# VisionDepth/VisionDepth3D

Hardware: AMD Instinct MI355X
Metric: stereo-pairs/sec end-to-end (depth+warp+fill+mux) (higher is better)
Workload: dtype f32

## Files before the change

### include/vd3d.h

```cpp
#ifndef VD3D_H
#define VD3D_H

#include <stddef.h>
#include <stdint.h>

#ifdef __cplusplus
extern "C" {
#endif

#define VD3D_ABI_VERSION 6

typedef enum vd3d_status {
  VD3D_OK = 0,
  VD3D_E_INVALID = -1,
  VD3D_E_HIP = -2,
  VD3D_E_NOMEM = -3,
  VD3D_E_UNSUPPORTED = -4
} vd3d_status;

typedef enum vd3d_format {
  VD3D_FMT_HALF_SBS = 0,
  VD3D_FMT_FULL_SBS = 1,
  VD3D_FMT_VR = 2,
  VD3D_FMT_ANAGLYPH = 3,
// ... 165 lines not shown
int vd3d_conv3x3_c64_f16(vd3d_ctx* ctx, const void* x_nhwc, int H, int W, const void* w_frag, const float* bias, const float* slope_or_null,
                         void* y_nhwc);
int vd3d_conv3x3_head_f16(vd3d_ctx* ctx, const void* x_nhwc3, int H, int W, const float* w27x64, const float* bias, const float* slope_or_null,
                          void* y_nhwc64);
int vd3d_esr_tail_f32(vd3d_ctx* ctx, const void* t_nhwc64, const void* x_nhwc3, int H, int W, int r, float* out_planar);

int vd3d_depth_handoff(vd3d_ctx* ctx, const float* pred, int B, int ph, int pw, int H, int W, int invert, uint8_t* out_gray);

typedef enum vd3d_dtype { VD3D_DT_BF16 = 0, VD3D_DT_F32 = 1, VD3D_DT_F16 = 2  } vd3d_dtype;

int vd3d_depth_preprocess(vd3d_ctx* ctx, const uint8_t* frames_bgr, int B, int H, int W, int th, int tw,
                          const float* mean3_host, const float* std3_host, int dtype, void* out_nhwc);

int vd3d_add_layernorm(vd3d_ctx* ctx, int dtype, const void* x, const void* y_or_null, const void* gamma, const void* beta,
                       float eps, int64_t rows, int cols, void* out_sum, void* out_norm);

enum { VD3D_GEMM_EPI_NONE = 0, VD3D_GEMM_EPI_GELU = 1 };
enum { VD3D_X3_BF16X3 = 0, VD3D_X3_FP16X2 = 1 };
int64_t vd3d_gemm_x3_weight_bytes(int N, int K, int mode);
int vd3d_gemm_x3_pack_weights(vd3d_ctx* ctx, const float* W, int N, int K, int mode, void* image);
int vd3d_gemm_x3(vd3d_ctx* ctx, const float* X, int64_t M, int K, const void* w_image, int N, int mode, const float* bias_or_null, int epilogue, float* Y);
int64_t vd3d_attention_x3_workspace_bytes(int B, int T, int H, int D, int mode);
int vd3d_attention_x3(vd3d_ctx* ctx, const float* qkv, int B, int T, int H, int D, float scale, int mode, void* workspace, int64_t workspace_bytes, float* out);

int64_t vd3d_conv3x3_x2_weight_bytes(int Cin, int Cout);
int vd3d_conv3x3_x2_pack_weights(vd3d_ctx* ctx, const float* W, int Cin, int Cout, void* image);
int vd3d_conv3x3_x2(vd3d_ctx* ctx, const float* X, int B, int H, int W, int Cin, const void* w_image, int Cout, float* Y);

int vd3d_upsample_bilinear_nhwc(vd3d_ctx* ctx, int dtype, const void* in, void* out, int B, int ih, int iw, int oh, int ow, int C);

int vd3d_nhwc_bias_act_f32(vd3d_ctx* ctx, const float* y, const float* bias_or_null, const float* r1_or_null, const float* r2_or_null, int relu,
                           int64_t n_pix, int C, float* out, float* relu_out_or_null);
int vd3d_upsample_bilinear_bias_nhwc_f32(vd3d_ctx* ctx, const float* in, const float* bias, float* out, int B, int ih, int iw, int oh, int ow, int C);
int vd3d_dpt_head_tail_f32(vd3d_ctx* ctx, const float* y, const float* b2, const float* w3, float b3, float scale, int64_t n_pix, int C, float* out);

int vd3d_depth_to_space_bias_nhwc_f32(vd3d_ctx* ctx, const float* y, const float* bias_or_null, int B, int H, int W, int s, int C, float* out);

typedef enum vd3d_preview {
  VD3D_PREVIEW_INTERLACED = 0,
  VD3D_PREVIEW_HSBS = 1,
  VD3D_PREVIEW_LR_DIFF = 2,
  VD3D_PREVIEW_FEATHER_BLEND = 3,
  VD3D_PREVIEW_RED_BLUE = 4
} vd3d_preview;
int vd3d_preview_image(vd3d_ctx* ctx, int type, const uint8_t* left_bgr, const uint8_t* right_bgr, int h, int w, uint8_t* out_bgr);
int vd3d_preview_heatmap(vd3d_ctx* ctx, int type, const float* shift_map, int h, int w, const uint8_t* lut_bgr_dev, uint8_t* out_bgr);
// ... 25 lines not shown
```

### visiondepth3d_amd/_lib.py

```python
from __future__ import annotations

import ctypes as C
import os

from . import _abi
from ._abi import FrameScalars, RenderParams, ShiftParams, State

_HERE = os.path.dirname(os.path.abspath(__file__))
LIB_PATH = os.environ.get("VD3D_LIB_PATH") or os.path.join(_HERE, "libvd3d_hip.so")

EXPORTS = (
    "vd3d_abi_version", "vd3d_last_error", "vd3d_shift_params_default", "vd3d_render_params_default",
    "vd3d_ctx_create", "vd3d_ctx_destroy", "vd3d_sync", "vd3d_ctx_stream", "vd3d_ctx_set_stream", "vd3d_ctx_pixel_stream", "vd3d_ctx_pixel_stream_k",
    "vd3d_state_reset", "vd3d_state_new_clip", "vd3d_state_export", "vd3d_state_import", "vd3d_state_planes",
    "vd3d_last_scalars", "vd3d_pixel_shift", "vd3d_render_frame", "vd3d_render_frame_blank", "vd3d_depth_handoff", "vd3d_heal_missing_pixels", "vd3d_preview_heatmap", "vd3d_preview_arrows", "vd3d_conv3x3_c64_f16", "vd3d_conv3x3_head_f16", "vd3d_esr_tail_f32", "vd3d_nv12_to_bgr", "vd3d_bgr_to_nv12", "vd3d_resize_cubic_u8", "vd3d_resize_area_u8", "vd3d_resize_linear_u8", "vd3d_format_3d_output", "vd3d_esr_preprocess", "vd3d_esr_postprocess", "vd3d_add_weighted_u8", "vd3d_rife_preprocess", "vd3d_rife_postprocess",
    "vd3d_shard_begin", "vd3d_shard_pixels", "vd3d_shard_pixels_blank", "vd3d_tdf_plane_export", "vd3d_tdf_plane_import", "vd3d_set_pixel_overlap", "vd3d_join_pixels", "vd3d_wait_pixels", "vd3d_finish_frame", "vd3d_quantiles",
    "vd3d_subject_depth", "vd3d_shard2_p0", "vd3d_shard2_set_crops", "vd3d_shard2_p1", "vd3d_shard2_p1_batch", "vd3d_shard2_r1", "vd3d_shard2_p3", "vd3d_shard2_p3_batch", "vd3d_shard2_r2", "vd3d_depth_preprocess", "vd3d_add_layernorm", "vd3d_gemm_x3_weight_bytes", "vd3d_gemm_x3_pack_weights", "vd3d_gemm_x3", "vd3d_attention_x3_workspace_bytes", "vd3d_attention_x3", "vd3d_conv3x3_x2_weight_bytes", "vd3d_conv3x3_x2_pack_weights", "vd3d_conv3x3_x2", "vd3d_upsample_bilinear_nhwc", "vd3d_nhwc_bias_act_f32", "vd3d_upsample_bilinear_bias_nhwc_f32", "vd3d_dpt_head_tail_f32", "vd3d_depth_to_space_bias_nhwc_f32", "vd3d_preview_image", "vd3d_detect_black_bars", "vd3d_stream_copy", "vd3d_torch_math", "vd3d_torch_math_aten", "vd3d_debug_gaussian_kernel1d", "vd3d_debug_exp_torch", "vd3d_set_profiling", "vd3d_last_stage_ms", "vd3d_stage_calls",
    "vd3d_debug_planes", "vd3d_debug_tune",
)

_lib = None


class Vd3dError(RuntimeError):
    def __init__(self, code, msg):
        super().__init__(f"libvd3d_hip error {code}: {msg}")
        self.code = code


def lib():
    global _lib
    if _lib is not None:
        return _lib
    if not os.path.exists(LIB_PATH):
        raise ImportError(f"{LIB_PATH} not built: run `python -c 'import __graft_entry__ as g; g.build()'` "
                          "(hipcc --offload-arch=gfx950). There is no CPU fallback.")
    L = C.CDLL(LIB_PATH)
    vp, i32, f32p, u8p = C.c_void_p, C.c_int, C.c_void_p, C.c_void_p
    L.vd3d_abi_version.restype = i32
    L.vd3d_last_error.restype = C.c_char_p
# ... 41 lines not shown
    L.vd3d_esr_postprocess.argtypes = [vp, f32p, i32, i32, i32, i32, i32, i32, i32, u8p, C.c_longlong]
    L.vd3d_rife_preprocess.argtypes = [vp, i32, u8p, u8p, i32, i32, i32, vp]
    L.vd3d_rife_postprocess.argtypes = [vp, f32p, i32, i32, i32, u8p]
    L.vd3d_add_weighted_u8.argtypes = [vp, u8p, C.c_double, u8p, C.c_double, C.c_double, C.c_longlong, u8p]
    L.vd3d_finish_frame.argtypes = [vp, u8p, u8p, f32p, i32, i32, C.POINTER(RenderParams), C.c_double, i32, i32, u8p]
    L.vd3d_quantiles.argtypes = [vp, f32p, C.c_int64, C.POINTER(C.c_float), i32, C.POINTER(C.c_float)]
    L.vd3d_subject_depth.argtypes = [vp, f32p, i32, i32, C.POINTER(C.c_float)]
    L.vd3d_shard2_p0.argtypes = [vp, vp, vp, vp]
    L.vd3d_shard2_set_crops.argtypes = [vp, vp, i32]
    L.vd3d_shard2_p1.argtypes = [vp, vp, vp, i32, vp, i32, i32, vp]
    L.vd3d_shard2_p1_batch.argtypes = [vp, vp, vp, i32, vp, i32, i32, i32, vp]
    L.vd3d_shard2_p3_batch.argtypes = [vp, i32, i32, i32, vp, vp]
    L.vd3d_shard2_r1.argtypes = [vp, vp, i32]
    L.vd3d_shard2_p3.argtypes = [vp, i32, i32, vp, vp]
    L.vd3d_shard2_r2.argtypes = [vp, vp, C.POINTER(C.c_int), C.POINTER(C.c_uint8), i32, vp]
    L.vd3d_depth_preprocess.argtypes = [vp, vp, i32, i32, i32, i32, i32, C.POINTER(C.c_float), C.POINTER(C.c_float), i32, vp]
    L.vd3d_gemm_x3_weight_bytes.argtypes = [i32, i32, i32]
    L.vd3d_gemm_x3_weight_bytes.restype = C.c_int64
    L.vd3d_gemm_x3_pack_weights.argtypes = [vp, vp, i32, i32, i32, vp]
    L.vd3d_gemm_x3.argtypes = [vp, vp, C.c_int64, i32, vp, i32, i32, vp, i32, vp]
    L.vd3d_attention_x3_workspace_bytes.argtypes = [i32, i32, i32, i32, i32]
    L.vd3d_attention_x3_workspace_bytes.restype = C.c_int64
    L.vd3d_attention_x3.argtypes = [vp, vp, i32, i32, i32, i32, C.c_float, i32, vp, C.c_int64, vp]
    L.vd3d_conv3x3_x2_weight_bytes.argtypes = [i32, i32]
    L.vd3d_conv3x3_x2_weight_bytes.restype = C.c_int64
    L.vd3d_conv3x3_x2_pack_weights.argtypes = [vp, vp, i32, i32, vp]
    L.vd3d_conv3x3_x2.argtypes = [vp, vp, i32, i32, i32, i32, vp, i32, vp]
    L.vd3d_add_layernorm.argtypes = [vp, i32, vp, vp, vp, vp, C.c_float, C.c_int64, i32, vp, vp]
    L.vd3d_upsample_bilinear_nhwc.argtypes = [vp, i32, vp, vp, i32, i32, i32, i32, i32, i32]
    L.vd3d_nhwc_bias_act_f32.argtypes = [vp, vp, vp, vp, vp, i32, C.c_int64, i32, vp, vp]
    L.vd3d_upsample_bilinear_bias_nhwc_f32.argtypes = [vp, vp, vp, vp, i32, i32, i32, i32, i32, i32]
    L.vd3d_dpt_head_tail_f32.argtypes = [vp, vp, vp, vp, C.c_float, C.c_float, C.c_int64, i32, vp]
    L.vd3d_depth_to_space_bias_nhwc_f32.argtypes = [vp, vp, vp, i32, i32, i32, i32, i32, vp]
    L.vd3d_preview_image.argtypes = [vp, i32, vp, vp, i32, i32, vp]
    L.vd3d_detect_black_bars.argtypes = [vp, vp, i32, i32, C.POINTER(C.c_int), C.POINTER(C.c_int)]
    L.vd3d_stream_copy.argtypes = [vp, vp, vp, C.c_size_t]
    L.vd3d_torch_math.argtypes = [vp, i32, vp, C.c_float, vp, C.c_longlong]
    L.vd3d_torch_math_aten.argtypes = [vp, i32, vp, C.c_double, vp, C.c_longlong, i32]
    L.vd3d_debug_gaussian_kernel1d.argtypes = [i32, C.c_float, vp]
    L.vd3d_debug_exp_torch.argtypes = [vp, vp, C.c_longlong]
    L.vd3d_debug_tune.argtypes = [i32, i32]
    L.vd3d_set_profiling.argtypes = [vp, i32]
    L.vd3d_last_stage_ms.argtypes = [vp, C.c_char_p]
    L.vd3d_last_stage_ms.restype = C.c_float
    L.vd3d_stage_calls.argtypes = [vp, C.c_char_p]
    L.vd3d_stage_calls.restype = C.c_long
# ... 20 lines not shown
```

### visiondepth3d_amd/csrc/vd3d_api.hip

```cpp
#include <hip/hip_runtime.h>

#include <cmath>
#include <cstdarg>
#include <cstddef>
#include <cstdio>
#include <cstring>
#include <cstdlib>
#include <map>
#include <string>
#include <vector>

#include "vd3d_kernels.h"

#define VD3D_EXPORT extern "C" __attribute__((visibility("default")))

static thread_local char g_err[512] = "";
static int set_err(int code, const char* fmt, ...) {
  va_list ap;
  va_start(ap, fmt);
  vsnprintf(g_err, sizeof g_err, fmt, ap);
  va_end(ap);
  return code;
}
#define HIPCHK(x)                                                                                     \
// ... 1303 lines not shown
VD3D_EXPORT int vd3d_conv3x3_x2_pack_weights(vd3d_ctx* c, const float* W, int Cin, int Cout, void* image) {
  if (!c || !W || !image) return set_err(VD3D_E_INVALID, "bad argument");
  if (!vd_launch_conv3x3_x2_pack(c->stream, W, Cin, Cout, image))
    return set_err(VD3D_E_UNSUPPORTED, "conv3x3_x2: C_in %d must be a positive multiple of 16 and C_out %d one of 64, 128", Cin, Cout);
  HIPCHK(hipGetLastError());
  return 0;
}

VD3D_EXPORT int vd3d_conv3x3_x2(vd3d_ctx* c, const float* X, int B, int H, int W, int Cin, const void* w_image, int Cout, float* Y) {
  if (!c || !X || !w_image || !Y) return set_err(VD3D_E_INVALID, "bad argument");
  if (!vd_launch_conv3x3_x2(c->stream, X, B, H, W, Cin, w_image, Cout, Y))
    return set_err(VD3D_E_UNSUPPORTED, "conv3x3_x2: C_in %d (multiple of 16), C_out %d (64 | 128), B %d <= 65535, 16-byte aligned input and image", Cin, Cout, B);
  HIPCHK(hipGetLastError());
  return 0;
}

VD3D_EXPORT int64_t vd3d_attention_x3_workspace_bytes(int B, int T, int H, int D, int mode) { return (int64_t)vd_attn_x3_workspace_bytes(B, T, H, D, mode); }

VD3D_EXPORT int vd3d_attention_x3(vd3d_ctx* c, const float* qkv, int B, int T, int H, int D, float scale, int mode, void* workspace, int64_t workspace_bytes, float* out) {
  if (!c || !qkv || !workspace || !out) return set_err(VD3D_E_INVALID, "bad argument");
  const long long need = vd_attn_x3_workspace_bytes(B, T, H, D, mode);
  if (need < 0) return set_err(VD3D_E_UNSUPPORTED, "attention_x3: head size %d not built (64), an unknown mode %d or an empty shape (B %d T %d H %d)", D, mode, B, T, H);
  if (workspace_bytes < need) return set_err(VD3D_E_INVALID, "attention_x3: workspace of %lld bytes, %lld needed", (long long)workspace_bytes, need);
  if (!vd_launch_attn_x3(c->stream, qkv, B, T, H, D, scale, workspace, out, mode))
    return set_err(VD3D_E_UNSUPPORTED, "attention_x3: qkv / workspace / out must be 16-byte aligned, B * H <= 65535");
  HIPCHK(hipGetLastError());
  return 0;
}

VD3D_EXPORT int64_t vd3d_gemm_x3_weight_bytes(int N, int K, int mode) { return (int64_t)vd_gemm_x3_weight_bytes(N, K, mode); }

VD3D_EXPORT int vd3d_gemm_x3_pack_weights(vd3d_ctx* c, const float* W, int N, int K, int mode, void* image) {
  if (!c || !W || !image) return set_err(VD3D_E_INVALID, "bad argument");
  if (!vd_launch_gemm_x3_pack_w(c->stream, W, N, K, image, mode)) return set_err(VD3D_E_UNSUPPORTED, "gemm_x3: K %d must be a positive multiple of 16 (N %d), mode %d in {0, 1}", K, N, mode);
  HIPCHK(hipGetLastError());
  return 0;
}

VD3D_EXPORT int vd3d_gemm_x3(vd3d_ctx* c, const float* X, int64_t M, int K, const void* w_image, int N, int mode, const float* bias_or_null, int epilogue, float* Y) {
  if (!c || !X || !w_image || !Y || M < 1) return set_err(VD3D_E_INVALID, "bad argument");
  if (epilogue != VD3D_GEMM_EPI_NONE && epilogue != VD3D_GEMM_EPI_GELU) return set_err(VD3D_E_INVALID, "gemm_x3: unknown epilogue %d", epilogue);
  if (!vd_launch_gemm_x3(c->stream, X, (long long)M, K, w_image, N, bias_or_null, epilogue, Y, mode))
    return set_err(VD3D_E_UNSUPPORTED, "gemm_x3: K %d must be a positive multiple of 16, mode %d in {0, 1}, X and the weight image 16-byte aligned", K, mode);
  HIPCHK(hipGetLastError());
  return 0;
}

VD3D_EXPORT int vd3d_upsample_bilinear_nhwc(vd3d_ctx* c, int dtype, const void* in, void* out, int B, int ih, int iw, int oh, int ow, int C) {
// ... 205 lines not shown
```

### visiondepth3d_amd/csrc/vd3d_attn.hip

```cpp
#include "vd3d_dev.h"
#include "vd3d_kernels.h"

typedef short at_bf8 __attribute__((ext_vector_type(8)));
typedef float at_f16 __attribute__((ext_vector_type(16)));
typedef uint32_t at_u4 __attribute__((ext_vector_type(4)));

#define AT_D 64
#define AT_BQ 256
#define AT_BK 64
#define AT_NT 512
#define AT_NTERM(MODE) ((MODE) == 0 ? 3 : 2)
#define AT_TILE(MODE) (4 * AT_NTERM(MODE) * 2 * 64 * 16)
#define AT_STAGE(MODE) (2 * AT_TILE(MODE))
#define AT_NSTAGE 3
#define AT_LDS(MODE) (AT_NSTAGE * AT_STAGE(MODE))
#define AT_QBLK(MODE) (4 * AT_NTERM(MODE) * 2 * 32)
#define AT_QKV_SCALE 16.0f
#define AT_P_SCALE 1024.0f
#define AT_OP 272

struct vd_at_args {
  int B, H, T;
  int nq32, nkv, nqb;
  float c;
// ... 255 lines not shown
  __builtin_amdgcn_s_barrier();

  const float l_tot = l_half + __shfl_xor(l_half, 32, 64);
  const float inv = MODE == 1 ? 1.0f / (l_tot * (AT_P_SCALE * AT_QKV_SCALE)) : 1.0f / l_tot;
  uint8_t* ow = at_lds + wave * (32 * AT_OP);
#pragma unroll
  for (int dm = 0; dm < 2; ++dm)
#pragma unroll
    for (int g = 0; g < 4; ++g) {
      const float4 v4 = {oacc[dm][4 * g] * inv, oacc[dm][4 * g + 1] * inv, oacc[dm][4 * g + 2] * inv, oacc[dm][4 * g + 3] * inv};
      *reinterpret_cast<float4*>(ow + li * AT_OP + (32 * dm + 8 * g + 4 * kh) * 4) = v4;
    }
  asm volatile("s_waitcnt lgkmcnt(0)" ::: "memory");
  const int b = bh / a.H, h = bh - b * a.H;
#pragma unroll
  for (int i = 0; i < 8; ++i) {
    const int row = i * 4 + (lane >> 4), c4 = lane & 15;
    const int q = q0 + row;
    const float4 v4 = *reinterpret_cast<const float4*>(ow + row * AT_OP + c4 * 16);
    if (q < a.T) *reinterpret_cast<float4*>(out + (((size_t)b * a.T + q) * a.H + h) * AT_D + c4 * 4) = v4;
  }
}

static bool at_mode_ok(int mode) { return mode == 0 || mode == 1; }
long long vd_attn_x3_workspace_bytes(int B, int T, int H, int D, int mode) {
  if (B < 1 || T < 1 || H < 1 || D != AT_D || !at_mode_ok(mode)) return -1;
  const long long nq32 = (T + 31) / 32, nkv = (T + AT_BK - 1) / AT_BK;
  const long long qblk = mode == 0 ? AT_QBLK(0) : AT_QBLK(1), tile = mode == 0 ? AT_TILE(0) : AT_TILE(1);
  return (long long)B * H * (nq32 * qblk * 16 + 2 * nkv * tile);
}

template <int MODE>
static bool at_launch(hipStream_t s, const float* qkv, int B, int T, int H, float scale, void* ws, float* out) {
  static bool attr_set = false;
  if (!attr_set) {
    if (hipFuncSetAttribute(reinterpret_cast<const void*>(k_attn_bf16x3<MODE>), hipFuncAttributeMaxDynamicSharedMemorySize, AT_LDS(MODE)) != hipSuccess) return false;
    attr_set = true;
  }
  vd_at_args a;
  a.B = B; a.H = H; a.T = T;
  a.nq32 = (T + 31) / 32; a.nkv = (T + AT_BK - 1) / AT_BK; a.nqb = (T + AT_BQ - 1) / AT_BQ;
  a.c = scale * 1.44269504088896340736f;
  if (MODE == 1) a.c *= 1.0f / (AT_QKV_SCALE * AT_QKV_SCALE);
  uint4* Qimg = reinterpret_cast<uint4*>(ws);
  uint4* Kimg = Qimg + (size_t)B * H * a.nq32 * AT_QBLK(MODE);
  uint4* Vimg = Kimg + (size_t)B * H * a.nkv * (AT_TILE(MODE) / 16);
  const int rows_max = a.nkv * 64 > a.nq32 * 32 ? a.nkv * 64 : a.nq32 * 32;
  hipLaunchKernelGGL(k_attn_x3_prep<MODE>, dim3((unsigned)((rows_max * 8 + 255) / 256), (unsigned)(B * H), 3), dim3(256), 0, s, qkv, a, Qimg, Kimg, Vimg);
  const int groups = (B * H + 7) / 8;
  hipLaunchKernelGGL(k_attn_bf16x3<MODE>, dim3((unsigned)(8 * groups * a.nqb)), dim3(AT_NT), AT_LDS(MODE), s, Qimg, Kimg, Vimg, out, a);
  return true;
}

bool vd_launch_attn_x3(hipStream_t s, const float* qkv, int B, int T, int H, int D, float scale, void* ws, float* out, int mode) {
  if (vd_attn_x3_workspace_bytes(B, T, H, D, mode) < 0) return false;
  if ((reinterpret_cast<uintptr_t>(qkv) & 15) || (reinterpret_cast<uintptr_t>(ws) & 15) || (reinterpret_cast<uintptr_t>(out) & 15)) return false;
  if ((long long)B * H > 65535) return false;
  return mode == 0 ? at_launch<0>(s, qkv, B, T, H, scale, ws, out) : at_launch<1>(s, qkv, B, T, H, scale, ws, out);
}
```

### visiondepth3d_amd/csrc/vd3d_kernels.h

```cpp
#pragma once
#include <hip/hip_runtime.h>

#include "vd3d_work.h"

enum { VD_ST_A0 = 0, VD_ST_B0, VD_ST_A1, VD_ST_B1, VD_ST_A2, VD_ST_B2,
       VD_ST_AQ, VD_ST_BQ, VD_ST_BS };
#define PL_KMAX_HOST 129
#define DF_RMAX_HOST 15

#define VD_ETAB 8
struct vd_stage_args {
  int stage;
  int have_eye;
  int W, H;
  long long n_eye;
  long long n_crop;
  double ipd_factor;
  int shard;
  int shard_idx;
  float* q_out;
  long long* m_out;
  const int* crop_tab;
  const float* etab;
  int dbg;
// ... 136 lines not shown
                               const vd_finish_consts& fc, const vd_dev_work* w, float focal_override, int use_override,
                               int bar_width, int bar_side, uint8_t* L_out, uint8_t* R_out, const float* wtab);
#define VD_D4_WTAB_FLOATS (4 * 31 * 32)
bool vd_launch_sharp_fit(hipStream_t s, const uint8_t* gL, const uint8_t* gR, const vd3d_render_params& p, const vd_finish_consts& fc, uint8_t* out);
void vd_launch_sharp_mux(hipStream_t s, const uint8_t* gL, const uint8_t* gR, const vd3d_render_params& p,
                         const vd_finish_consts& fc, uint8_t* out, int presharp_pitch = 0, bool identity_fit = false);
void vd_launch_stream_copy(hipStream_t s, const void* src, void* dst, size_t bytes);
void vd_launch_interp_planes(hipStream_t s, const float* src, int C, int ih, int iw, float* dst, int oh, int ow, int premult);
void vd_launch_torch_math_aten(hipStream_t s, int op, const float* x, double p, float* out, long long n, int threads);
void vd_launch_torch_math(hipStream_t s, int op, const float* x, float p, float* out, long long n);
void vd_launch_blank_eye(hipStream_t s, const uint8_t* src, int h, int w, const vd_dev_work* wk, uint8_t* dst);

bool vd_launch_preview(hipStream_t s, int type, const uint8_t* L, const uint8_t* R, int h, int w, uint8_t* out);
bool vd_launch_depth_prep(hipStream_t s, const uint8_t* frames, int B, int H, int W, int th, int tw, const float mean[3],
                          const float stdv[3], int dtype, void* out_nhwc);
long long vd_gemm_x3_weight_bytes(int N, int K, int mode);
bool vd_launch_gemm_x3_pack_w(hipStream_t s, const float* W, int N, int K, void* img, int mode);
bool vd_launch_gemm_x3(hipStream_t s, const float* X, long long M, int K, const void* wimg, int N, const float* bias, int epilogue, float* Y, int mode);
long long vd_conv3x3_x2_weight_bytes(int Cin, int Cout);
bool vd_launch_conv3x3_x2_pack(hipStream_t s, const float* W, int Cin, int Cout, void* img);
bool vd_launch_conv3x3_x2(hipStream_t s, const float* X, int B, int H, int W, int Cin, const void* wimg, int Cout, float* Y);
long long vd_attn_x3_workspace_bytes(int B, int T, int H, int D, int mode);
bool vd_launch_attn_x3(hipStream_t s, const float* qkv, int B, int T, int H, int D, float scale, void* ws, float* out, int mode);
bool vd_launch_add_layernorm(hipStream_t s, int dtype, const void* x, const void* y, const void* gamma, const void* beta, float eps,
                             long long rows, int cols, void* out_sum, void* out_norm);
bool vd_launch_upsample_bilinear_nhwc(hipStream_t s, int dtype, const void* in, void* out, int B, int ih, int iw, int oh, int ow, int C);
bool vd_launch_bias_act_f32(hipStream_t s, const float* y, const float* bias, const float* r1, const float* r2, int relu, long long n_pix, int C,
                            float* out, float* relu_out);
bool vd_launch_upsample_bilinear_bias_nhwc_f32(hipStream_t s, const float* in, const float* bias, float* out, int B, int ih, int iw, int oh, int ow, int C);
bool vd_launch_head_tail_f32(hipStream_t s, const float* y, const float* b2, const float* w3, float b3, float scale, long long n_pix, int C, float* out);
bool vd_launch_depth_to_space_bias_f32(hipStream_t s, const float* y, const float* bias, int B, int H, int W, int f, int C, float* out);
void vd_launch_depth_handoff(hipStream_t s, const float* pred, int B, int ph, int pw, int H, int W, int invert, uint32_t* mm,
                             uint8_t* out);

bool vd_launch_finish_fused(hipStream_t s, const uint8_t* L, const uint8_t* R, const float* dn, int eh, int ew,
                            const vd3d_render_params& p, const vd_finish_consts& fc, const vd_dev_work* w, float focal,
                            int use_override, int bar_w, int bar_s, uint8_t* out, int dense, const float* w2_dev);

bool vd_launch_conv3x3_c64_f16(hipStream_t s, const void* x, int H, int W, const void* wfrag, const float* bias, const float* slope_or_null, void* y);
void vd_launch_conv3x3_head_f16(hipStream_t s, const void* x, int H, int W, const float* w27, const float* bias, const float* slope_or_null, void* y);
void vd_launch_esr_tail_f32(hipStream_t s, const void* t, const void* x, int H, int W, int r, float* out);
void vd_launch_nv12_to_bgr(hipStream_t s, const uint8_t* y, const uint8_t* uv, int h, int w, long long y_pitch, long long uv_pitch, uint8_t* out);
void vd_launch_bgr_to_nv12(hipStream_t s, const uint8_t* bgr, int h, int w, uint8_t* y, uint8_t* uv, long long y_pitch, long long uv_pitch);
bool vd_launch_preview_heatmap(hipStream_t s, int type, const float* shift, int h, int w, const uint8_t* lut_dev, uint32_t* mm, uint8_t* out);
void vd_launch_preview_arrows(hipStream_t s, const uint8_t* left, const float* shift, int h, int w, uint8_t* out);
bool vd_launch_resize_cubic_u8(hipStream_t s, const uint8_t* src, int sh, int sw, int cn, uint8_t* dst, int dh, int dw);
// ... 10 lines not shown
```

### visiondepth3d_amd/depth.py

```python
from __future__ import annotations

import json
import os
import zlib

import numpy as np
import torch
import torch.nn.functional as F

_DA_S = dict(arch="da", hidden=384, layers=12, heads=6, out_indices=[9, 10, 11, 12], neck=[48, 96, 192, 384], fusion=64, head=32)
_DA_B = dict(arch="da", hidden=768, layers=12, heads=12, out_indices=[9, 10, 11, 12], neck=[96, 192, 384, 768], fusion=128, head=32)
_DA_L = dict(arch="da", hidden=1024, layers=24, heads=16, out_indices=[21, 22, 23, 24], neck=[256, 512, 1024, 1024], fusion=256, head=32)
MODEL_ZOO = {
    "depth-anything-v2-small": _DA_S, "depth-anything-v2-base": _DA_B, "depth-anything-v2-large": _DA_L,
    "depth-anything-v1-small": _DA_S, "depth-anything-v1-base": _DA_B, "depth-anything-v1-large": _DA_L,
    "distill-any-depth-small": _DA_S, "distill-any-depth-large": _DA_L,
    "dpt-large": dict(arch="dpt", hidden=1024, layers=24, heads=16, out_indices=[5, 11, 17, 23], neck=[256, 512, 1024, 1024], fusion=256),
}
IMAGENET_MEAN = (0.485, 0.456, 0.406)
IMAGENET_STD = (0.229, 0.224, 0.225)
PROCESSORS = {
    "da": dict(size=(518, 518), keep_aspect_ratio=True, multiple=14, mean=IMAGENET_MEAN, std=IMAGENET_STD),
    "dpt": dict(size=(384, 384), keep_aspect_ratio=False, multiple=1, mean=(0.5, 0.5, 0.5), std=(0.5, 0.5, 0.5)),
}
# ... 394 lines not shown
            wo = (out.weight.float() * l1[:, None]).to(out.weight.dtype).contiguous()
            bo = (out.bias.float() * l1).to(out.bias.dtype).contiguous()
            fc1, fc2 = layer.mlp.fc1, layer.mlp.fc2
            w2 = (fc2.weight.float() * l2[:, None]).to(fc2.weight.dtype).contiguous()
            b2 = (fc2.bias.float() * l2).to(fc2.bias.dtype).contiguous()
            nh, hd, scaling = att.num_attention_heads, att.attention_head_size, att.scaling
            n1, n2, act = layer.norm1, layer.norm2, layer.mlp.activation
            nxt = layers[li + 1].norm1 if li + 1 < len(layers) else None
            x3 = None
            if self.gemm != "f32":
                x3 = self._split_block(stash, pad_state, wqkv, bqkv, wo, bo, fc1.weight, fc1.bias, w2, b2, nh, hd, scaling, n1, n2, act, nxt)

            def fwd(x, wqkv=wqkv, bqkv=bqkv, wo=wo, bo=bo, fc1=fc1, w2=w2, b2=b2, nh=nh, hd=hd, scaling=scaling, n1=n1, n2=n2,
                    act=act, nxt=nxt, x3=x3):
                if x3 is not None:
                    return x3(x)
                B, T, d = x.shape
                hip = R is not None and x.dtype in (torch.bfloat16, torch.float32) and x.is_contiguous() and d in (384, 768, 1024)
                if hip:
                    h = stash["h"] if stash["x"] is x else R.add_layernorm(x, None, n1)[1]
                    stash["x"] = stash["h"] = None
                else:
                    h = n1(x)
                qkv = F.linear(h, wqkv, bqkv).view(B, T, 3, nh, hd)
                Tk = pad_state["T"] or T
                q, k, v = qkv[:, :, 0].transpose(1, 2), qkv[:, :Tk, 1].transpose(1, 2), qkv[:, :Tk, 2].transpose(1, 2)
                o = F.scaled_dot_product_attention(q, k, v, scale=scaling).transpose(1, 2).reshape(B, T, d)
                a = F.linear(o, wo, bo)
                if not hip:
                    x = x + a
                    return x + F.linear(act(fc1(n2(x))), w2, b2)
                x, h = R.add_layernorm(x, a, n2)
                m = F.linear(act(fc1(h)), w2, b2)
                if nxt is None:
                    return x + m
                x, hn = R.add_layernorm(x, m, nxt)
                stash["x"], stash["h"] = x, hn
                return x

            layer.forward = fwd

    def _split_block(self, stash, pad_state, wqkv, bqkv, wo, bo, w1, b1, w2, b2, nh, hd, scaling, n1, n2, act, nxt):
        R, gm = self.renderer, self.gemm
        gelu_ok = isinstance(act, torch.nn.GELU) and getattr(act, "approximate", "none") == "none" or type(act).__name__ == "GELUActivation"
        x3 = dict(qkv=(R.gemm_x3_pack(wqkv, gm), wqkv.shape[0]), wo=(R.gemm_x3_pack(wo, gm), wo.shape[0]),
                  fc1=(R.gemm_x3_pack(w1, gm), w1.shape[0]), w2=(R.gemm_x3_pack(w2, gm), w2.shape[0]), gelu=bool(gelu_ok), mode=gm)

        def lin(t, key, bias, gelu=False):
            return R.linear_x3(t if t.is_contiguous() else t.contiguous(), x3[key][0], x3[key][1], bias, gelu=gelu, mode=gm)

# ... 185 lines not shown
```

### visiondepth3d_amd/render_3d.py

```python
from __future__ import annotations

import ctypes as C

import numpy as np
import torch

from . import _lib
from ._abi import DEPTH_BGR_U8, DEPTH_F32, DEPTH_GRAY_U8, DT_BF16, DT_F16, DT_F32, FORMAT_IDS, FrameScalars, RenderParams, ShiftParams, State
from .geometry import aspect_ratios
from .params import reference_aten_threads, render_kwargs_to_params, shift_params_from_kwargs

torch_device = torch.device("cuda" if torch.cuda.is_available() else "cpu")


def _ptr(t: torch.Tensor):
    return C.c_void_p(t.data_ptr())


class Renderer:

    def __init__(self, device: int | torch.device | None = None, private_stream: bool = False, auto_order: bool = True):
        if not torch.cuda.is_available():
            raise RuntimeError("visiondepth3d_amd needs a ROCm GPU (MI355X); there is no CPU path")
        L = _lib.lib()
# ... 516 lines not shown
        K = x.shape[-1]
        M = x.numel() // K
        out = torch.empty(x.shape[:-1] + (int(N),), dtype=torch.float32, device=x.device)
        self._enter(x, w_image, bias, out)
        _lib.check(self._L.vd3d_gemm_x3(self._ctx, _ptr(x), M, K, _ptr(w_image), int(N), self.X3_MODES[mode], _ptr(bias) if bias is not None else None,
                                        1 if gelu else 0, _ptr(out)))
        return out

    def attention_x3(self, qkv: torch.Tensor, n_heads: int, scale: float, mode: str = "bf16x3") -> torch.Tensor:
        B, T, C3 = qkv.shape
        D = C3 // (3 * n_heads)
        if qkv.dtype != torch.float32 or not qkv.is_contiguous() or D * 3 * n_heads != C3:
            raise AssertionError("qkv must be contiguous float32 [B, T, 3 * H * D]")
        m = self.X3_MODES[mode]
        nb = int(self._L.vd3d_attention_x3_workspace_bytes(B, T, n_heads, D, m))
        if nb < 0:
            raise NotImplementedError(f"attention_x3: head size {D} not built")
        ws = getattr(self, "_attn_ws", None)
        if ws is None or ws.numel() < nb:
            ws = self._attn_ws = torch.empty(nb, dtype=torch.uint8, device=self.device)
        out = torch.empty((B, T, n_heads * D), dtype=torch.float32, device=self.device)
        self._enter(qkv, ws, out)
        _lib.check(self._L.vd3d_attention_x3(self._ctx, _ptr(qkv), B, T, n_heads, D, float(scale), m, _ptr(ws), ws.numel(), _ptr(out)))
        return out

    def conv3x3_x2_pack(self, weight: torch.Tensor):
        w = weight.detach().to(self.device, torch.float32).contiguous()
        Cout, Cin, kh, kw = w.shape
        nb = int(self._L.vd3d_conv3x3_x2_weight_bytes(Cin, Cout)) if (kh, kw) == (3, 3) else -1
        if nb < 0:
            return None
        img = torch.empty(nb, dtype=torch.uint8, device=self.device)
        self._enter(w, img)
        _lib.check(self._L.vd3d_conv3x3_x2_pack_weights(self._ctx, _ptr(w), Cin, Cout, _ptr(img)))
        return img

    def conv3x3_x2(self, x: torch.Tensor, w_image: torch.Tensor, Cout: int) -> torch.Tensor:
        B, Cin, H, W = x.shape
        if x.dtype != torch.float32 or not x.is_contiguous(memory_format=torch.channels_last):
            raise AssertionError("conv3x3_x2: float32 channels_last input")
        out = torch.empty((B, int(Cout), H, W), dtype=torch.float32, device=x.device, memory_format=torch.channels_last)
        self._enter(x, w_image, out)
        _lib.check(self._L.vd3d_conv3x3_x2(self._ctx, _ptr(x), B, H, W, Cin, _ptr(w_image), int(Cout), _ptr(out)))
        return out

    def upsample_bilinear(self, x: torch.Tensor, size) -> torch.Tensor:
# ... 193 lines not shown
```

Measured before the change: 133.5.

## Add fused f32 flash-attention kernel on MFMA for unpadded depth blocks

Adds a new HIP flash-attention kernel that reads the packed qkv tensor directly, stages K/V tiles into LDS with async global-to-LDS loads over three stages, and computes QK^T and PV with fp32 MFMA and an online softmax. The depth model's attention path now calls this kernel instead of PyTorch SDPA when the input is f32 with head size 64 and no padding. This removes the q/k/v transpose views and SDPA dispatch, keeping full f32 precision. LDS opt-in is also made per-device.

```diff
diff --git a/include/vd3d.h b/include/vd3d.h
--- a/include/vd3d.h
+++ b/include/vd3d.h
@@ -211,6 +211,7 @@
 int vd3d_gemm_x3(vd3d_ctx* ctx, const float* X, int64_t M, int K, const void* w_image, int N, int mode, const float* bias_or_null, int epilogue, float* Y);
 int64_t vd3d_attention_x3_workspace_bytes(int B, int T, int H, int D, int mode);
 int vd3d_attention_x3(vd3d_ctx* ctx, const float* qkv, int B, int T, int H, int D, float scale, int mode, void* workspace, int64_t workspace_bytes, float* out);
+int vd3d_attention_f32(vd3d_ctx* ctx, const float* qkv, int B, int T, int H, int D, float scale, float* out);
 
 int64_t vd3d_conv3x3_x2_weight_bytes(int Cin, int Cout);
 int vd3d_conv3x3_x2_pack_weights(vd3d_ctx* ctx, const float* W, int Cin, int Cout, void* image);
diff --git a/visiondepth3d_amd/_lib.py b/visiondepth3d_amd/_lib.py
--- a/visiondepth3d_amd/_lib.py
+++ b/visiondepth3d_amd/_lib.py
@@ -15,7 +15,7 @@
     "vd3d_state_reset", "vd3d_state_new_clip", "vd3d_state_export", "vd3d_state_import", "vd3d_state_planes",
     "vd3d_last_scalars", "vd3d_pixel_shift", "vd3d_render_frame", "vd3d_render_frame_blank", "vd3d_depth_handoff", "vd3d_heal_missing_pixels", "vd3d_preview_heatmap", "vd3d_preview_arrows", "vd3d_conv3x3_c64_f16", "vd3d_conv3x3_head_f16", "vd3d_esr_tail_f32", "vd3d_nv12_to_bgr", "vd3d_bgr_to_nv12", "vd3d_resize_cubic_u8", "vd3d_resize_area_u8", "vd3d_resize_linear_u8", "vd3d_format_3d_output", "vd3d_esr_preprocess", "vd3d_esr_postprocess", "vd3d_add_weighted_u8", "vd3d_rife_preprocess", "vd3d_rife_postprocess",
     "vd3d_shard_begin", "vd3d_shard_pixels", "vd3d_shard_pixels_blank", "vd3d_tdf_plane_export", "vd3d_tdf_plane_import", "vd3d_set_pixel_overlap", "vd3d_join_pixels", "vd3d_wait_pixels", "vd3d_finish_frame", "vd3d_quantiles",
-    "vd3d_subject_depth", "vd3d_shard2_p0", "vd3d_shard2_set_crops", "vd3d_shard2_p1", "vd3d_shard2_p1_batch", "vd3d_shard2_r1", "vd3d_shard2_p3", "vd3d_shard2_p3_batch", "vd3d_shard2_r2", "vd3d_depth_preprocess", "vd3d_add_layernorm", "vd3d_gemm_x3_weight_bytes", "vd3d_gemm_x3_pack_weights", "vd3d_gemm_x3", "vd3d_attention_x3_workspace_bytes", "vd3d_attention_x3", "vd3d_conv3x3_x2_weight_bytes", "vd3d_conv3x3_x2_pack_weights", "vd3d_conv3x3_x2", "vd3d_upsample_bilinear_nhwc", "vd3d_nhwc_bias_act_f32", "vd3d_upsample_bilinear_bias_nhwc_f32", "vd3d_dpt_head_tail_f32", "vd3d_depth_to_space_bias_nhwc_f32", "vd3d_preview_image", "vd3d_detect_black_bars", "vd3d_stream_copy", "vd3d_torch_math", "vd3d_torch_math_aten", "vd3d_debug_gaussian_kernel1d", "vd3d_debug_exp_torch", "vd3d_set_profiling", "vd3d_last_stage_ms", "vd3d_stage_calls",
+    "vd3d_subject_depth", "vd3d_shard2_p0", "vd3d_shard2_set_crops", "vd3d_shard2_p1", "vd3d_shard2_p1_batch", "vd3d_shard2_r1", "vd3d_shard2_p3", "vd3d_shard2_p3_batch", "vd3d_shard2_r2", "vd3d_depth_preprocess", "vd3d_add_layernorm", "vd3d_gemm_x3_weight_bytes", "vd3d_gemm_x3_pack_weights", "vd3d_gemm_x3", "vd3d_attention_x3_workspace_bytes", "vd3d_attention_x3", "vd3d_attention_f32", "vd3d_conv3x3_x2_weight_bytes", "vd3d_conv3x3_x2_pack_weights", "vd3d_conv3x3_x2", "vd3d_upsample_bilinear_nhwc", "vd3d_nhwc_bias_act_f32", "vd3d_upsample_bilinear_bias_nhwc_f32", "vd3d_dpt_head_tail_f32", "vd3d_depth_to_space_bias_nhwc_f32", "vd3d_preview_image", "vd3d_detect_black_bars", "vd3d_stream_copy", "vd3d_torch_math", "vd3d_torch_math_aten", "vd3d_debug_gaussian_kernel1d", "vd3d_debug_exp_torch", "vd3d_set_profiling", "vd3d_last_stage_ms", "vd3d_stage_calls",
     "vd3d_debug_planes", "vd3d_debug_tune",
 )
 
@@ -103,6 +103,7 @@
     L.vd3d_attention_x3_workspace_bytes.argtypes = [i32, i32, i32, i32, i32]
     L.vd3d_attention_x3_workspace_bytes.restype = C.c_int64
     L.vd3d_attention_x3.argtypes = [vp, vp, i32, i32, i32, i32, C.c_float, i32, vp, C.c_int64, vp]
+    L.vd3d_attention_f32.argtypes = [vp, vp, i32, i32, i32, i32, C.c_float, vp]
     L.vd3d_conv3x3_x2_weight_bytes.argtypes = [i32, i32]
     L.vd3d_conv3x3_x2_weight_bytes.restype = C.c_int64
     L.vd3d_conv3x3_x2_pack_weights.argtypes = [vp, vp, i32, i32, vp]
diff --git a/visiondepth3d_amd/csrc/vd3d_api.hip b/visiondepth3d_amd/csrc/vd3d_api.hip
--- a/visiondepth3d_amd/csrc/vd3d_api.hip
+++ b/visiondepth3d_amd/csrc/vd3d_api.hip
@@ -1349,8 +1349,18 @@
   const long long need = vd_attn_x3_workspace_bytes(B, T, H, D, mode);
   if (need < 0) return set_err(VD3D_E_UNSUPPORTED, "attention_x3: head size %d not built (64), an unknown mode %d or an empty shape (B %d T %d H %d)", D, mode, B, T, H);
   if (workspace_bytes < need) return set_err(VD3D_E_INVALID, "attention_x3: workspace of %lld bytes, %lld needed", (long long)workspace_bytes, need);
+  HIPCHK(hipSetDevice(c->device));
   if (!vd_launch_attn_x3(c->stream, qkv, B, T, H, D, scale, workspace, out, mode))
     return set_err(VD3D_E_UNSUPPORTED, "attention_x3: qkv / workspace / out must be 16-byte aligned, B * H <= 65535");
+  HIPCHK(hipGetLastError());
+  return 0;
+}
+
+VD3D_EXPORT int vd3d_attention_f32(vd3d_ctx* c, const float* qkv, int B, int T, int H, int D, float scale, float* out) {
+  if (!c || !qkv || !out) return set_err(VD3D_E_INVALID, "bad argument");
+  HIPCHK(hipSetDevice(c->device));
+  if (!vd_launch_attn_f32(c->stream, qkv, B, T, H, D, scale, out))
+    return set_err(VD3D_E_UNSUPPORTED, "attention_f32: head size %d not built (64), an empty shape (B %d T %d H %d), B * H > 65535 or qkv / out not 16-byte aligned", D, B, T, H);
   HIPCHK(hipGetLastError());
   return 0;
 }
diff --git a/visiondepth3d_amd/csrc/vd3d_attn.hip b/visiondepth3d_amd/csrc/vd3d_attn.hip
--- a/visiondepth3d_amd/csrc/vd3d_attn.hip
+++ b/visiondepth3d_amd/csrc/vd3d_attn.hip
@@ -1,5 +1,7 @@
 #include "vd3d_dev.h"
 #include "vd3d_kernels.h"
+
+#include <mutex>
 
 typedef short at_bf8 __attribute__((ext_vector_type(8)));
 typedef float at_f16 __attribute__((ext_vector_type(16)));
@@ -301,6 +303,177 @@
   }
 }
 
+#define AF_TILE (AT_BK * AT_D * 4)
+#define AF_STAGE (2 * AF_TILE)
+#define AF_LDS (AT_NSTAGE * AF_STAGE)
+VD_DEV void af_st(const uint8_t* __restrict__ sk, const float (&qf)[32], int li, int kh, at_f16 (&s)[2]) {
+  const int kswz = (li & 15) << 4;
+#pragma unroll
+  for (int m = 0; m < 2; ++m)
+#pragma unroll
+    for (int r = 0; r < 16; ++r) s[m][r] = 0.f;
+#pragma unroll
+  for (int g = 0; g < 8; ++g) {
+    float4 kf[2];
+#pragma unroll
+    for (int m = 0; m < 2; ++m) kf[m] = *reinterpret_cast<const float4*>(sk + (32 * m + li) * 256 + (((8 * kh + g) << 4) ^ kswz));
+#pragma unroll
+    for (int m = 0; m < 2; ++m) s[m] = __builtin_amdgcn_mfma_f32_32x32x2f32(kf[m].x, qf[4 * g], s[m], 0, 0, 0);
+#pragma unroll
+    for (int m = 0; m < 2; ++m) s[m] = __builtin_amdgcn_mfma_f32_32x32x2f32(kf[m].y, qf[4 * g + 1], s[m], 0, 0, 0);
+#pragma unroll
+    for (int m = 0; m < 2; ++m) s[m] = __builtin_amdgcn_mfma_f32_32x32x2f32(kf[m].z, qf[4 * g + 2], s[m], 0, 0, 0);
+#pragma unroll
+    for (int m = 0; m < 2; ++m) s[m] = __builtin_amdgcn_mfma_f32_32x32x2f32(kf[m].w, qf[4 * g + 3], s[m], 0, 0, 0);
+  }
+}
+VD_DEV void af_pv(const uint8_t* __restrict__ sv, const at_f16 (&p)[2], int li, int kh, at_f16 (&oacc)[2]) {
+#pragma unroll
+  for (int m = 0; m < 2; ++m)
+#pragma unroll
+    for (int r = 0; r < 16; ++r) {
+      const float2 vv = *reinterpret_cast<const float2*>(sv + (32 * m + (r & 3) + 8 * (r >> 2) + 4 * kh) * 256 + li * 8);
+      oacc[0] = __builtin_amdgcn_mfma_f32_32x32x2f32(vv.x, p[m][r], oacc[0], 0, 0, 0);
+      oacc[1] = __builtin_amdgcn_mfma_f32_32x32x2f32(vv.y, p[m][r], oacc[1], 0, 0, 0);
+    }
+}
+
+__global__ __launch_bounds__(AT_NT) void k_attn_f32(const float* __restrict__ qkv, float* __restrict__ out, vd_at_args a) {
+  extern __shared__ __attribute__((aligned(16))) uint8_t at_lds[];
+  int bh, qb;
+  {
+    const int wg = blockIdx.x, x = wg & 7, idx = wg >> 3;
+    const int g = idx / a.nqb;
+    qb = idx - g * a.nqb;
+    bh = g * 8 + x;
+    if (bh >= a.B * a.H) return;
+  }
+  const int tid = threadIdx.x, lane = tid & 63, wave = __builtin_amdgcn_readfirstlane(tid >> 6);
+  const int li = lane & 31, kh = lane >> 5;
+  const int q0 = qb * AT_BQ + wave * 32;
+  const int b = bh / a.H, h = bh - b * a.H;
+  const size_t tok_stride = (size_t)3 * a.H * AT_D;
+  const float* base = qkv + (size_t)b * a.T * tok_stride + h * AT_D;
+
+  const int drow = tid >> 4, dpos = tid & 15, kchunk = dpos ^ (drow & 15);
+  auto dma = [&](int tile, int stage) {
+    uint8_t* dst = at_lds + stage * AF_STAGE + wave * 1024;
+#pragma unroll
+    for (int p = 0; p < 2; ++p) {
+      const int tok = min(tile * AT_BK + drow + 32 * p, a.T - 1);
+      const float* src = base + (size_t)tok * tok_stride + a.H * AT_D;
+      __builtin_amdgcn_global_load_lds((at_glb_vp)(src + kchunk * 4), (at_lds_vp)(dst + p * 8192), 16, 0, 0);
+      __builtin_amdgcn_global_load_lds((at_glb_vp)(src + a.H * AT_D + dpos * 4), (at_lds_vp)(dst + AF_TILE + p * 8192), 16, 0, 0);
+    }
+  };
+
+  float qf[32];
+  {
+    const float4* qp = reinterpret_cast<const float4*>(base + (size_t)min(q0 + li, a.T - 1) * tok_stride + 32 * kh);
+#pragma unroll
+    for (int g = 0; g < 8; ++g) {
+      const float4 v = qp[g];
+      qf[4 * g] = v.x * a.c; qf[4 * g + 1] = v.y * a.c; qf[4 * g + 2] = v.z * a.c; qf[4 * g + 3] = v.w * a.c;
+    }
+  }
+  dma(0, 0);
+  if (a.nkv > 1) {
+    dma(1, 1);
+    asm volatile("s_waitcnt vmcnt(4)" ::: "memory");
+  } else {
+    asm volatile("s_waitcnt vmcnt(0)" ::: "memory");
+  }
+  __builtin_amdgcn_s_barrier();
+
+  at_f16 oacc[2];
+#pragma unroll
+  for (int dm = 0; dm < 2; ++dm)
+#pragma unroll
+    for (int r = 0; r < 16; ++r) oacc[dm][r] = 0.f;
+  float m_run = -INFINITY, l_half = 0.f;
+  int cur = 0;
+  for (int it = 0; it < a.nkv; ++it) {
+    const bool ahead = it + 2 < a.nkv;
+    if (ahead) dma(it + 2, cur == 0 ? 2 : cur - 1);
+    const uint8_t* sk = at_lds + cur * AF_STAGE;
+    const uint8_t* sv = sk + AF_TILE;
+    at_f16 s[2];
+    af_st(sk, qf, li, kh, s);
+    if ((it + 1) * AT_BK > a.T) {
+#pragma unroll
+      for (int m = 0; m < 2; ++m)
+#pragma unroll
+        for (int r = 0; r < 16; ++r)
+          if (it * AT_BK + 32 * m + (r & 3) + 8 * (r >> 2) + 4 * kh >= a.T) s[m][r] = -INFINITY;
+    }
+    float mx = s[0][0];
+#pragma unroll
+    for (int m = 0; m < 2; ++m)
+#pragma unroll
+      for (int r = 0; r < 16; ++r) mx = fmaxf(mx, s[m][r]);
+    mx = fmaxf(mx, __shfl_xor(mx, 32, 64));
+    const float m_new = fmaxf(m_run, mx);
+    if (__any(m_new > m_run)) {
+      const float alpha = __builtin_amdgcn_exp2f(m_run - m_new);
+#pragma unroll
+      for (int dm = 0; dm < 2; ++dm)
+#pragma unroll
+        for (int r = 0; r < 16; ++r) oacc[dm][r] *= alpha;
+      l_half *= alpha;
+      m_run = m_new;
+    }
+    float ps = 0.f;
+#pragma unroll
+    for (int m = 0; m < 2; ++m)
+#pragma unroll
+      for (int r = 0; r < 16; ++r) { s[m][r] = __builtin_amdgcn_exp2f(s[m][r] - m_run); ps += s[m][r]; }
+    l_half += ps;
+    af_pv(sv, s, li, kh, oacc);
+    if (ahead) asm volatile("s_waitcnt vmcnt(4) lgkmcnt(0)" ::: "memory"); else asm volatile("s_waitcnt vmcnt(0) lgkmcnt(0)" ::: "memory");
+    __builtin_amdgcn_s_barrier();
+    cur = cur == 2 ? 0 : cur + 1;
+  }
+
+  const float l_tot = l_half + __shfl_xor(l_half, 32, 64);
+  const int q = q0 + li;
+  if (q < a.T) {
+    float* op = out + (((size_t)b * a.T + q) * a.H + h) * AT_D + 8 * kh;
+#pragma unroll
+    for (int g = 0; g < 4; ++g) {
+      const float4 lo = {oacc[0][4 * g] / l_tot, oacc[1][4 * g] / l_tot, oacc[0][4 * g + 1] / l_tot, oacc[1][4 * g + 1] / l_tot};
+      const float4 hi = {oacc[0][4 * g + 2] / l_tot, oacc[1][4 * g + 2] / l_tot, oacc[0][4 * g + 3] / l_tot, oacc[1][4 * g + 3] / l_tot};
+      *reinterpret_cast<float4*>(op + 16 * g) = lo;
+      *reinterpret_cast<float4*>(op + 16 * g + 4) = hi;
+    }
+  }
+}
+
+static bool at_lds_optin(const void* fn, int lds, bool (&done)[64]) {
+  static std::mutex mu;
+  int dev = 0;
+  if (hipGetDevice(&dev) != hipSuccess || dev < 0 || dev >= 64) return false;
+  std::lock_guard<std::mutex> lock(mu);
+  if (!done[dev]) {
+    if (hipFuncSetAttribute(fn, hipFuncAttributeMaxDynamicSharedMemorySize, lds) != hipSuccess) return false;
+    done[dev] = true;
+  }
+  return true;
+}
+
+bool vd_launch_attn_f32(hipStream_t s, const float* qkv, int B, int T, int H, int D, float scale, float* out) {
+  if (B < 1 || T < 1 || H < 1 || D != AT_D || (long long)B * H > 65535) return false;
+  if ((reinterpret_cast<uintptr_t>(qkv) & 15) || (reinterpret_cast<uintptr_t>(out) & 15)) return false;
+  static bool attr_set[64] = {};
+  if (!at_lds_optin(reinterpret_cast<const void*>(k_attn_f32), AF_LDS, attr_set)) return false;
+  vd_at_args a;
+  a.B = B; a.H = H; a.T = T;
+  a.nq32 = (T + 31) / 32; a.nkv = (T + AT_BK - 1) / AT_BK; a.nqb = (T + AT_BQ - 1) / AT_BQ;
+  a.c = scale * 1.44269504088896340736f;
+  const int groups = (B * H + 7) / 8;
+  hipLaunchKernelGGL(k_attn_f32, dim3((unsigned)(8 * groups * a.nqb)), dim3(AT_NT), AF_LDS, s, qkv, out, a);
+  return true;
+}
+
 static bool at_mode_ok(int mode) { return mode == 0 || mode == 1; }
 long long vd_attn_x3_workspace_bytes(int B, int T, int H, int D, int mode) {
   if (B < 1 || T < 1 || H < 1 || D != AT_D || !at_mode_ok(mode)) return -1;
@@ -311,11 +484,8 @@
 
 template <int MODE>
 static bool at_launch(hipStream_t s, const float* qkv, int B, int T, int H, float scale, void* ws, float* out) {
-  static bool attr_set = false;
-  if (!attr_set) {
-    if (hipFuncSetAttribute(reinterpret_cast<const void*>(k_attn_bf16x3<MODE>), hipFuncAttributeMaxDynamicSharedMemorySize, AT_LDS(MODE)) != hipSuccess) return false;
-    attr_set = true;
-  }
+  static bool attr_set[64] = {};
+  if (!at_lds_optin(reinterpret_cast<const void*>(k_attn_bf16x3<MODE>), AT_LDS(MODE), attr_set)) return false;
   vd_at_args a;
   a.B = B; a.H = H; a.T = T;
   a.nq32 = (T + 31) / 32; a.nkv = (T + AT_BK - 1) / AT_BK; a.nqb = (T + AT_BQ - 1) / AT_BQ;
diff --git a/visiondepth3d_amd/csrc/vd3d_kernels.h b/visiondepth3d_amd/csrc/vd3d_kernels.h
--- a/visiondepth3d_amd/csrc/vd3d_kernels.h
+++ b/visiondepth3d_amd/csrc/vd3d_kernels.h
@@ -182,6 +182,7 @@
 bool vd_launch_conv3x3_x2(hipStream_t s, const float* X, int B, int H, int W, int Cin, const void* wimg, int Cout, float* Y);
 long long vd_attn_x3_workspace_bytes(int B, int T, int H, int D, int mode);
 bool vd_launch_attn_x3(hipStream_t s, const float* qkv, int B, int T, int H, int D, float scale, void* ws, float* out, int mode);
+bool vd_launch_attn_f32(hipStream_t s, const float* qkv, int B, int T, int H, int D, float scale, float* out);
 bool vd_launch_add_layernorm(hipStream_t s, int dtype, const void* x, const void* y, const void* gamma, const void* beta, float eps,
                              long long rows, int cols, void* out_sum, void* out_norm);
 bool vd_launch_upsample_bilinear_nhwc(hipStream_t s, int dtype, const void* in, void* out, int B, int ih, int iw, int oh, int ow, int C);
diff --git a/visiondepth3d_amd/depth.py b/visiondepth3d_amd/depth.py
--- a/visiondepth3d_amd/depth.py
+++ b/visiondepth3d_amd/depth.py
@@ -440,10 +440,14 @@
                     stash["x"] = stash["h"] = None
                 else:
                     h = n1(x)
-                qkv = F.linear(h, wqkv, bqkv).view(B, T, 3, nh, hd)
-                Tk = pad_state["T"] or T
-                q, k, v = qkv[:, :, 0].transpose(1, 2), qkv[:, :Tk, 1].transpose(1, 2), qkv[:, :Tk, 2].transpose(1, 2)
-                o = F.scaled_dot_product_attention(q, k, v, scale=scaling).transpose(1, 2).reshape(B, T, d)
+                qkv = F.linear(h, wqkv, bqkv)
+                if R is not None and x.dtype == torch.float32 and hd == 64 and not pad_state["T"]:
+                    o = R.attention_f32(qkv, nh, scaling)
+                else:
+                    qkv = qkv.view(B, T, 3, nh, hd)
+                    Tk = pad_state["T"] or T
+                    q, k, v = qkv[:, :, 0].transpose(1, 2), qkv[:, :Tk, 1].transpose(1, 2), qkv[:, :Tk, 2].transpose(1, 2)
+                    o = F.scaled_dot_product_attention(q, k, v, scale=scaling).transpose(1, 2).reshape(B, T, d)
                 a = F.linear(o, wo, bo)
                 if not hip:
                     x = x + a
diff --git a/visiondepth3d_amd/render_3d.py b/visiondepth3d_amd/render_3d.py
--- a/visiondepth3d_amd/render_3d.py
+++ b/visiondepth3d_amd/render_3d.py
@@ -562,6 +562,18 @@
         out = torch.empty((B, T, n_heads * D), dtype=torch.float32, device=self.device)
         self._enter(qkv, ws, out)
         _lib.check(self._L.vd3d_attention_x3(self._ctx, _ptr(qkv), B, T, n_heads, D, float(scale), m, _ptr(ws), ws.numel(), _ptr(out)))
+        return out
+
+    def attention_f32(self, qkv: torch.Tensor, n_heads: int, scale: float) -> torch.Tensor:
+        B, T, C3 = qkv.shape
+        D = C3 // (3 * n_heads)
+        if qkv.dtype != torch.float32 or not qkv.is_contiguous() or D * 3 * n_heads != C3:
+            raise AssertionError("qkv must be contiguous float32 [B, T, 3 * H * D]")
+        if D != 64:
+            raise NotImplementedError(f"attention_f32: head size {D} not built")
+        out = torch.empty((B, T, n_heads * D), dtype=torch.float32, device=self.device)
+        self._enter(qkv, out)
+        _lib.check(self._L.vd3d_attention_f32(self._ctx, _ptr(qkv), B, T, n_heads, D, float(scale), _ptr(out)))
         return out
 
     def conv3x3_x2_pack(self, weight: torch.Tensor):
```

Measured after the change: 138.9, median of 6. +4.1%, better.
